# ArisKonidaris/OMLDM

Hardware: AMD Instinct MI355X
Metric: training examples/sec (whole node) + p50 predict latency, linear SVM 1/2/4/8 GPU (higher is better)
Workload: dtype fp32

## Files before the change

csrc/kernels/linear_scan3.hip:

```cpp
#include "common.h"
#include "hash_dev.h"
#include "seq_common.h"

#include <mutex>
#include <unordered_map>

namespace omldm {

typedef float f32x4 __attribute__((ext_vector_type(4)));

namespace s3 {
constexpr int CH = 64;
#ifndef OMLDM_S3_NH
#define OMLDM_S3_NH 11
#endif
constexpr int NH = OMLDM_S3_NH;
constexpr int NT = 64 * (NH + 1);
constexpr int WPE = (NH + 1 + 3) / 4;
constexpr int NHA = NH;
constexpr int GS = CH + 4;
constexpr int MAXF = 32;
constexpr int NF = (MAXF + NHA - 1) / NHA;
constexpr int KNMAX = 32;
constexpr int NJ = (KNMAX + NHA - 1) / NHA;
// ... 762 lines not shown
  const int n = cb.lidcount[s];
  const float sc = cb.inv_p * (cb.sig ? cb.sig[s] : 1.f);
  const int* l2 = cb.l2s + (size_t)s * cb.gs;
  constexpr int FB = 8;
  for (int i0 = threadIdx.x; i0 < n; i0 += FB * s3::NT) {
    int slot[FB];
    float d[FB];
#pragma unroll
    for (int u = 0; u < FB; ++u) {
      const int i = i0 + u * s3::NT;
      slot[u] = l2[i < n ? i : 0];
    }
#pragma unroll
    for (int u = 0; u < FB; ++u) {
      const int i = i0 + u * s3::NT;
      d[u] = i < min(n, cap) ? tab[i] : 0.f;
    }
    if (n > cap) {
#pragma unroll
      for (int u = 0; u < FB; ++u) {
        const int i = i0 + u * s3::NT;
        if (i >= cap && i < n)
          d[u] = __hip_atomic_load(&ag[i - cap], __ATOMIC_RELAXED, __HIP_MEMORY_SCOPE_AGENT);
      }
    }
    if constexpr (!RARE) {
#pragma unroll
      for (int u = 0; u < FB; ++u) {
        const int i = i0 + u * s3::NT;
        const int sl = i < n ? slot[u] : 0;
        d[u] -= i < n ? (cb.wbf ? s3_w16(w, sl) : w[sl]) : 0.f;
      }
    }
#pragma unroll
    for (int u = 0; u < FB; ++u) {
      const int i = i0 + u * s3::NT;
      if (i < n && d[u] != 0.f) atomicAdd(&cb.dacc[slot[u]], sc * d[u]);
    }
  }
}

__device__ __forceinline__ void s3_spoke_end(bool tail, const int* __restrict__ slotsT, int dc,
                                             int B, int R, const S3Comb& cb,
                                             const float* __restrict__ ws,
                                             const float* __restrict__ wsd, int dn, int dim,
                                             const SeqParams& p, S3Smem& sm, int s) {
  if (tail) {
    __syncthreads();
    s3_combine_spoke(slotsT, dc, B, R, cb, sm, s, 0, 1);
  }
  s3_scan_arrive(cb, ws, wsd, dn, dim, p, sm);
}

template <int RULE, int KN, bool RARE>
__device__ __forceinline__ void s3_scan_body(
    int bid, int nblk, int tail, S3Smem& sm, float* tab,
    const int* __restrict__ slotsT, const uint32_t* __restrict__ meta, int dc, int dn,
    const void* __restrict__ yv, int B, int R, const float* __restrict__ prep, int nchs,
    const float* __restrict__ w, int dim, float* __restrict__ aglob, int cap, long long gstride,
    const S3Comb& cb, float* __restrict__ ws, float* __restrict__ wsd, const SeqParams& p,
    unsigned long long* __restrict__ rgran) {
  constexpr int PF = s3_prep_floats<KN>();
  if (bid >= cb.S_act) {
    if (RARE && bid < 2 * cb.S_act) {
      s3_rare(slotsT, dc, B, R, w, cb, rgran, sm, bid - cb.S_act);
      if (cb.inscan == 2) s3_fold_pres(meta, dc, B, R, cb, bid - cb.S_act);
      if (tail == 2) {
        __syncthreads();
        s3_combine_spoke(slotsT, dc, B, R, cb, sm, bid - cb.S_act, 0, 1);
      }
      return;
    }
    s3_combine(slotsT, dc, B, R, cb, sm, (RARE ? 2 : 1) * cb.S_act, bid, nblk, cb.cns);
    return;
  }
  const int tid = threadIdx.x;
  const int wave = __builtin_amdgcn_readfirstlane(tid >> 6), lane = tid & 63;
  const int s = bid;
  int t0, t1;
  spoke_rows(s, R, B, t0, t1);
  if (t0 >= t1) {
    if (tid < s3::WS) ws[(size_t)s * s3::WS + tid] = 0.f;
    if (tid < s3::DS) wsd[(size_t)s * s3::DS + tid] = 0.f;
    s3_scan_arrive(cb, ws, wsd, dn, dim, p, sm);
    return;
  }
  const int nch = (t1 - t0 + s3::CH - 1) / s3::CH;
  const float* P0 = prep + (size_t)s * nchs * PF;
  auto chunk_prep = [&](int k) { return P0 + (size_t)k * PF; };
  float* ag = aglob + (size_t)s * gstride;

  unsigned long long* stamps = g_s3_stamps;
  const bool dbg_gather = g_s3_debug == 1;
  unsigned long long st_acc[12] = {};
  unsigned long long st_t = stamps ? clock64() : 0;
  auto stamp = [&](int k) {
    if (stamps) {
      const unsigned long long now = clock64();
      st_acc[k] += now - st_t;
      st_t = now;
    }
  };

  if (wave == 0) {
    __builtin_amdgcn_s_setprio(3);
    float loss = 0.f, nex = 0.f, mist = 0.f, sqe = 0.f;
    float f1 = 0.f;
    float ynx = chunk_prep(0)[s3_prep_y<KN>() + lane];
    float anx = chunk_prep(0)[2 * s3::MAT + lane];
    const bool shr = p.shr != 0;
    float snx = shr ? chunk_prep(0)[s3_prep_sg<KN>() + lane] : 1.f;
    float hnx = shr ? chunk_prep(0)[s3_prep_hh<KN>() + lane] : 1.f;
    for (int k = -1; k <= nch; ++k) {
      if (k >= 0 && k < nch) {
        const int b = k & 1;
        const int row = t0 + k * s3::CH + lane;
        const bool valid = row < t1 && ynx == ynx;
        const float y = valid ? ynx : 0.f;
        const float a = valid ? anx : 0.f;
        const float sg = valid ? snx : 1.f, hh = valid ? hnx : 1.f;
        if (k + 1 < nch) {
          ynx = chunk_prep(k + 1)[s3_prep_y<KN>() + lane];
          anx = chunk_prep(k + 1)[2 * s3::MAT + lane];
          if (shr) {
            snx = chunk_prep(k + 1)[s3_prep_sg<KN>() + lane];
            hnx = chunk_prep(k + 1)[s3_prep_hh<KN>() + lane];
          }
        }
        float m0 = 0.f;
#pragma unroll
        for (int q = 0; q < s3::NHA; ++q) m0 += sm.part[b][q][lane];
        S3Cand<RULE> cf;
        float u, bc = 0.f;
        const float inv = -a;
        if constexpr (RULE == kSeqHinge) {
          bc = y * inv * hh;
          cf.lo = y < 0.f ? -p.cclip * hh : 0.f;
          cf.hi = y < 0.f ? 0.f : (y > 0.f ? p.cclip * hh : 0.f);
          u = fmaf(a * (sg * hh), m0, bc) + f1;
        } else if constexpr (RULE == kSeqEps) {
          bc = (y - p.eps) * inv * hh;
          cf.d = 2.f * p.eps * inv * hh;
          cf.lo = valid ? -p.cclip * hh : 0.f;
          cf.hi = valid ? p.cclip * hh : 0.f;
          u = fmaf(a * (sg * hh), m0, bc) + f1;
        } else if constexpr (RULE == kSeqPegasos) {
          const float T = p.tbase + (float)(row - t0);
          cf.lo = valid ? 1.f / sg : 0.f;
          cf.hi = valid ? y * hh / (p.lam * T) : 0.f;
          u = fmaf(a, m0, 0.f) + f1;
        } else {
          cf.lo = y * sg;
          cf.hi = p.lr * y * hh;
          u = m0 + f1;
        }
        const float* grow = &sm.G[b][lane][0];
        const float* xrow = &sm.X1[b ^ 1][lane][0];
        float gg[s3::CH], xx[s3::CH];
#pragma unroll
        for (int t4 = 0; t4 < s3::CH; t4 += 4) {
          const float4 g4 = *reinterpret_cast<const float4*>(grow + t4);
          const float4 x4 = *reinterpret_cast<const float4*>(xrow + t4);
          gg[t4] = g4.x, gg[t4 + 1] = g4.y, gg[t4 + 2] = g4.z, gg[t4 + 3] = g4.w;
          xx[t4] = x4.x, xx[t4 + 1] = x4.y, xx[t4 + 2] = x4.z, xx[t4 + 3] = x4.w;
        }
        stamp(8);
        float n1 = 0.f;
        auto chain = [&](auto step) {
#pragma unroll
          for (int t = 0; t < s3::CH; ++t) {
            const float ct = readlane_f(step(u), t);
            u = fmaf(ct, gg[t], u);
            n1 = fmaf(ct, xx[t], n1);
            asm volatile("" : "+v"(u), "+v"(n1));
          }
        };
        if constexpr (RULE == kSeqLogistic) {
          if (!shr) {
            const float lo2 = y * 1.44269504088896341f;
            chain([&](float v) {
              return __builtin_amdgcn_rcpf(1.f + __builtin_amdgcn_exp2f(lo2 * v));
            });
          } else {
            chain([&](float v) { return cf(v, p, y); });
          }
        } else {
          chain([&](float v) { return cf(v, p, y); });
        }
        stamp(9);
        const float c = cf(u, p, y);
        sm.cb[b][lane] = c;
        if (row < t1 && cb.inscan != 1)
          __hip_atomic_store((s3_gu64*)(cb.gran + row),
                             ((unsigned long long)cb.epoch << 32) | __float_as_uint(c),
                             __ATOMIC_RELAXED, __HIP_MEMORY_SCOPE_AGENT);
        if (valid) {
          float m;
          if constexpr (RULE == kSeqLogistic) m = sg * u;
          else if constexpr (RULE == kSeqPegasos) m = sg * y * u;
          else m = inv > 0.f ? (bc - u) * __builtin_amdgcn_rcpf(inv * hh) : 0.f;
          seq_stats<RULE>(m, y, p, loss, mist, sqe);
          nex += 1.f;
        }
        f1 = n1;
      }
      stamp(0);
      __syncthreads();
      stamp(1);
    }
    if (stamps && lane == 0)
      for (int q = 0; q < 12; ++q)
        if (q < 2 || q >= 8) atomicAdd(&stamps[(size_t)s * 16 + q], st_acc[q]);
    loss = wave_sum(loss);
    nex = wave_sum(nex);
    mist = wave_sum(mist);
    sqe = wave_sum(sqe);
    if (lane == 0) {
      float* wr = ws + (size_t)s * s3::WS;
      wr[0] = loss;
      wr[1] = nex;
      wr[2] = mist;
      wr[3] = sqe;
      wr[4] = 1.f;
      wr[5] = 0.f;
      wr[6] = 0.f;
      wr[7] = 0.f;
    }
    if (cb.inscan) s3_inscan_flush<RARE>(cb, tab, ag, cap, w, s);
    s3_spoke_end(tail == 1, slotsT, dc, B, R, cb, ws, wsd, dn, dim, p, sm, s);
    return;
  }

  const int q = wave - 1, r = lane;
  const int swave = g_s3_debug >= 16 ? g_s3_debug - 16 : 1;
  if (g_s3_hprio) {
    if (q >= 7) __builtin_amdgcn_s_setprio(2);
    else if (q >= 3) __builtin_amdgcn_s_setprio(1);
  }
  const int qd = g_s3_dense_order ? s3::NHA - 1 - q : q;
  const int kd = dn + (p.bias ? 1 : 0);
  const int hl = q * 64 + lane;
  const bool inscan = cb.inscan != 0, inscan1 = cb.inscan == 1;
  const uint32_t tmask = inscan ? s3::F_TAB : s3::F_SCAT;
  const float isc = inscan1 ? cb.inv_p * (cb.sig ? cb.sig[s] : 1.f) : 0.f;
  float wn[s3::NJ], w0[s3::NJ];
#pragma unroll
  for (int i = 0; i < s3::NJ; ++i) {
    const int j = qd + s3::NHA * i;
    const int jw = j < dn ? j : dim - 1;
    const float wj = cb.wbf ? s3_w16(w, jw) : w[jw];
    w0[i] = (j < KN && (j < dn || (p.bias && j == dn))) ? wj : 0.f;
    wn[i] = w0[i];
  }
  constexpr int NV4 = (2 * s3::MAT / 4 + 64 * s3::NHA - 1) / (64 * s3::NHA);
  struct Set {
    int cs[s3::NF];
    uint32_t cm[s3::NF];
    float g[s3::NF];
    f32x4 v[NV4];
    float xs[s3::NJ], xc[s3::NJ];
    unsigned long long rg;
  };
  uint32_t p1[s3::NF], p2[s3::NF];
  const unsigned long long want = (unsigned long long)cb.epoch;
  bool dead = false;
  auto load_rare = [&](int ch) -> unsigned long long {
    const int row = t0 + ch * s3::CH + r;
    const bool ok = RARE && q == 0 && ch >= 0 && ch < nch && row < t1;
    return ok ? __hip_atomic_load((s3_gu64*)(rgran + row), __ATOMIC_RELAXED,
                                  __HIP_MEMORY_SCOPE_AGENT)
              : (want << 32);
  };
  auto load_words = [&](int ch, Set& S) {
    if constexpr (RARE) {
      S.rg = load_rare(ch);
#pragma unroll
      for (int i = 0; i < s3::NF; ++i) {
        const int f = q + s3::NHA * i;
        const int row = t0 + ch * s3::CH + r;
        const bool ok = ch >= 0 && ch < nch && f < dc && row < t1;
        const uint32_t mm = meta[ok ? (size_t)f * B + row : 0];
        S.cm[i] = ok ? mm : 0u;
        S.cs[i] = ok && (mm & (s3::F_TG | s3::F_INIT)) ? 0 : -1;
      }
      return;
    }
#pragma unroll
    for (int i = 0; i < s3::NF; ++i) {
      const int f = q + s3::NHA * i;
      const int row = t0 + ch * s3::CH + r;
      const bool ok = ch >= 0 && ch < nch && f < dc && row < t1;
      const size_t at = ok ? (size_t)f * B + row : 0;
      const int sl = slotsT[at];
      const uint32_t mm = meta[at];
      S.cs[i] = ok ? sl : -1;
      S.cm[i] = ok ? mm : 0u;
    }
  };
  auto issue_gathers = [&](Set& S) {
    if constexpr (RARE) return;
    if (cb.wbf) {
#pragma unroll
      for (int i = 0; i < s3::NF; ++i) {
        const bool glob = !RARE && S.cs[i] != -1 && !(S.cm[i] & s3::F_TG);
        S.g[i] = s3_w16(w, (glob && !dbg_gather) ? (S.cs[i] & 0x7fffffff) : 0);
      }
      return;
    }
#pragma unroll
    for (int i = 0; i < s3::NF; ++i) {
      const bool glob = !RARE && S.cs[i] != -1 && !(S.cm[i] & s3::F_TG);
      S.g[i] = w[(glob && !dbg_gather) ? (S.cs[i] & 0x7fffffff) : 0];
    }
  };
  auto issue_staging = [&](int ch, Set& S) {
#pragma unroll
    for (int u = 0; u < NV4; ++u) {
      const int i = min(hl + 64 * s3::NHA * u, 2 * s3::MAT / 4 - 1);
      const int mtx = i >> 10, e = i & 1023;
      const int kc = max(0, min(ch + mtx, nch - 1));
      S.v[u] = reinterpret_cast<const f32x4*>(chunk_prep(kc) + mtx * s3::MAT)[e];
    }
  };
  constexpr int NJK = (KN + s3::NHA - 1) / s3::NHA;
  auto load_dense = [&](int ch, float* xd) {
#pragma unroll
    for (int i = 0; i < NJK; ++i) {
      const int j = qd + s3::NHA * i;
      const bool ok = j < KN && ch >= 0 && ch < nch;
      const int jc = j < KN ? j : 0, cc = max(0, min(ch, nch - 1));
      const float v = chunk_prep(cc)[2 * s3::MAT + s3::CH + jc * s3::CH + r];
      xd[i] = ok ? v : 0.f;
    }
  };
  auto body = [&](auto spill_tag, int k, Set& CUR, Set& NXT) {
    constexpr bool SPILL = decltype(spill_tag)::value;
    const int cn = k + 1, ks = k - 1;
    if (wave == swave) stamp(7);
    load_words(cn + 1, NXT);
    issue_staging(cn + 1, NXT);
    load_dense(ks + 1, NXT.xs);
    load_dense(cn + 1, NXT.xc);
    if (wave == swave) stamp(3);
    if (ks >= 0) {
      const float cv = sm.cb[ks & 1][r];
#pragma unroll
      for (int i = 0; i < s3::NF; ++i) {
        const uint32_t m = p2[i];
        const bool sc = (m & tmask) != 0u && cv != 0.f;
        const bool dr = inscan1 && (m & s3::F_PRES) != 0u && cv != 0.f;
        if (__builtin_amdgcn_ballot_w64(sc || dr) == 0ull) continue;
        const int lid = (int)(m >> s3::LID_SHIFT);
        const float val = (m & s3::F_SIGN) ? -cv : cv;
        if (dr) atomicAdd(&cb.dacc[lid], val * isc);
        if (sc) {
          if constexpr (SPILL) {
            if (lid < cap) atomicAdd(&tab[lid], val);
            else atomicAdd(&ag[lid - cap], val);
          } else {
            atomicAdd(&tab[lid], val);
          }
        }
      }
#pragma unroll
      for (int i = 0; i < NJK; ++i) {
        const int j = qd + s3::NHA * i;
        if (j < kd) wn[i] += wave_sum(cv * CUR.xs[i]);
      }
    }
    if (wave == swave) stamp(6);
    if (cn < nch) {
      float base = 0.f;
#pragma unroll
      for (int i = 0; i < NJK; ++i) base = fmaf(CUR.xc[i], wn[i], base);
      if constexpr (RARE) {
        if (q == 0) {
          for (unsigned spins = 0;
               __builtin_amdgcn_ballot_w64((CUR.rg >> 32) != want) != 0ull;) {
            if (dead || ++spins > s3::SPIN_MAX) {
              if (!dead && r == 0) atomicExch(&g_s3_comb_err, 2);
              dead = true;
              break;
            }
            __builtin_amdgcn_s_sleep(1);
            CUR.rg = load_rare(cn);
          }
          base += (CUR.rg >> 32) == want ? __uint_as_float((uint32_t)CUR.rg) : 0.f;
        }
      }
      if constexpr (!SPILL) {
        float tv[s3::NF];
#pragma unroll
        for (int i = 0; i < s3::NF; ++i) {
          const uint32_t m = CUR.cm[i];
          const bool tg = CUR.cs[i] != -1 && (m & s3::F_TG);
          tv[i] = 0.f;
          if (tg) tv[i] = tab[(int)(m >> s3::LID_SHIFT)];
        }
#pragma unroll
        for (int i = 0; i < s3::NF; ++i) {
          const uint32_t m = CUR.cm[i];
          const bool here = CUR.cs[i] != -1;
          const bool tg = here && (m & s3::F_TG), init = here && !tg && (m & s3::F_INIT);
          const float val = tg ? tv[i] : (RARE ? 0.f : CUR.g[i]);
          if (init) tab[(int)(m >> s3::LID_SHIFT)] = val;
          if (here && (!RARE || tg)) base += (m & s3::F_SIGN) ? -val : val;
        }
      }
#pragma unroll
      for (int i = 0; SPILL && i < s3::NF; ++i) {
        const uint32_t m = CUR.cm[i];
        const bool here = CUR.cs[i] != -1;
        const int lid = (int)(m >> s3::LID_SHIFT);
        const bool tg = here && (m & s3::F_TG), init = here && !tg && (m & s3::F_INIT);
        float val = RARE ? 0.f : CUR.g[i];
        if (!SPILL || __builtin_amdgcn_ballot_w64((tg || init) && lid >= cap) == 0ull) {
          if (tg) val = tab[lid];
          if (init) tab[lid] = val;
        } else if constexpr (SPILL) {
          if (tg) val = lid < cap ? tab[lid] : __hip_atomic_load(&ag[lid - cap], __ATOMIC_RELAXED,
                                                                 __HIP_MEMORY_SCOPE_WORKGROUP);
          if (init) {
            if (lid < cap) tab[lid] = val;
            else __hip_atomic_store(&ag[lid - cap], val, __ATOMIC_RELAXED,
                                    __HIP_MEMORY_SCOPE_WORKGROUP);
          }
          asm volatile("s_waitcnt vmcnt(0)" ::: "memory");
        }
        if (here && (!RARE || tg)) base += (m & s3::F_SIGN) ? -val : val;
      }
      sm.part[cn & 1][q][r] = base;
    }
    if (wave == swave) stamp(4);
#pragma unroll
    for (int u = 0; u < NV4; ++u) {
      const int i = hl + 64 * s3::NHA * u;
      const int mtx = i >> 10, e = i & 1023;
      if (i < 2 * s3::MAT / 4 && cn + mtx < nch) {
        const int row = e >> 4, col = (e & 15) * 4;
        float* dst = mtx == 0 ? &sm.G[cn & 1][row][col] : &sm.X1[(cn + 1) & 1][row][col];
        *reinterpret_cast<f32x4*>(dst) = CUR.v[u];
      }
    }
    issue_gathers(NXT);
#pragma unroll
    for (int i = 0; i < s3::NF; ++i) {
      p2[i] = p1[i];
      p1[i] = CUR.cm[i];
    }
    if (wave == swave) stamp(5);
    __syncthreads();
  };

  Set A, Bs;
#pragma unroll
  for (int i = 0; i < s3::NF; ++i) p1[i] = p2[i] = 0u;
  load_words(0, A);
  issue_staging(0, A);
  load_dense(-2, A.xs);
  load_dense(0, A.xc);
  issue_gathers(A);
  if (cb.lidcount[s] <= cap) {
    for (int k = -1; k <= nch; k += 2) {
      body(S3Tag<false>{}, k, A, Bs);
      if (k + 1 <= nch) body(S3Tag<false>{}, k + 1, Bs, A);
    }
  } else {
    for (int k = -1; k <= nch; k += 2) {
      body(S3Tag<true>{}, k, A, Bs);
      if (k + 1 <= nch) body(S3Tag<true>{}, k + 1, Bs, A);
    }
  }
  if (stamps && lane == 0 && wave == swave)
    for (int k = 2; k < 8; ++k) atomicAdd(&stamps[(size_t)s * 16 + k], st_acc[k]);
#pragma unroll
  for (int i = 0; i < s3::NJ; ++i) {
    const int j = qd + s3::NHA * i;
    if (lane == 0 && j < KN) wsd[(size_t)s * s3::DS + j] = wn[i] - w0[i];
  }
  if (q == 0 && lane >= KN && lane < s3::DS) wsd[(size_t)s * s3::DS + lane] = 0.f;
  if (cb.inscan) s3_inscan_flush<RARE>(cb, tab, ag, cap, w, s);
  s3_spoke_end(tail == 1, slotsT, dc, B, R, cb, ws, wsd, dn, dim, p, sm, s);
}

constexpr int kS3MaxPipes = 16;
struct S3Pipe {
  const float* w;
  float* aglob;
  float* ws;
  float* wsd;
  unsigned long long* rgran;
  S3Comb cb;
  SeqParams p;
};
struct S3Pipes {
  int M;
  int ncomb;
  int tail;
  const unsigned long long* wflag;
  unsigned long long wepoch;
  S3Pipe pipe[kS3MaxPipes];
};

__global__ void s3_signal_kernel(unsigned long long* flag, unsigned long long epoch) {
  if (threadIdx.x == 0)
    __hip_atomic_store(flag, epoch, __ATOMIC_RELEASE, __HIP_MEMORY_SCOPE_AGENT);
}

__device__ __forceinline__ void s3_wait_prep(const unsigned long long* flag,
                                             unsigned long long epoch) {
  if (flag == nullptr) return;
  if (threadIdx.x == 0) {
    for (unsigned spins = 0;
         __hip_atomic_load(flag, __ATOMIC_RELAXED, __HIP_MEMORY_SCOPE_AGENT) < epoch;) {
      if (++spins > s3::SPIN_MAX) {
        atomicExch(&g_s3_comb_err, 3);
        break;
      }
      __builtin_amdgcn_s_sleep(2);
    }
    __builtin_amdgcn_fence(__ATOMIC_ACQUIRE, "agent");
  }
  __syncthreads();
}

template <int RULE, int KN, bool RARE>
__global__ __launch_bounds__(s3::NT, s3::WPE) __attribute__((amdgpu_waves_per_eu(s3::WPE, s3::WPE))) void s3_scan_kernel(
    const int* __restrict__ slotsT, const uint32_t* __restrict__ meta, int dc, int dn,
    const void* __restrict__ yv, int B, int R, const float* __restrict__ prep, int nchs,
    int dim, int cap, long long gstride, int S_act, S3Pipes pp) {
  __shared__ S3Smem sm;
  extern __shared__ float tab[];
  const int nblk = s3_nper(S_act, RARE, pp.ncomb, pp.pipe[0].cb.cns);
  const int pi = (int)blockIdx.x / nblk, local = (int)blockIdx.x % nblk;
  s3_wait_prep(pp.wflag, pp.wepoch);
  int bid;
  if (RARE && local < S_act) bid = S_act + local;
  else if (RARE && local < 2 * S_act) bid = local - S_act;
  else bid = local;
  const S3Pipe& P = pp.pipe[pi];
  s3_scan_body<RULE, KN, RARE>(bid, nblk, pp.tail, sm, tab, slotsT, meta,
                               dc, dn, yv, B, R, prep, nchs, P.w, dim, P.aglob, cap, gstride,
                               P.cb, P.ws, P.wsd, P.p, P.rgran);
}

__device__ void s3_dense_body(const float* __restrict__ ws,
                              const float* __restrict__ wsd, const float* __restrict__ sig,
                              int S_act, int dn, int dim, int bias, float inv_p,
                              float* __restrict__ dacc,
                              double* __restrict__ cum) {
  const int tid = threadIdx.x;
  const bool bad = __hip_atomic_load(&g_s3_comb_err, __ATOMIC_RELAXED, __HIP_MEMORY_SCOPE_AGENT) != 0;
  for (int i = tid; i < dn; i += 256) {
    float v = 0.f;
    for (int s = 0; s < S_act; ++s) v += wsd[(size_t)s * s3::DS + i] * (sig ? sig[s] : 1.f);
    dacc[i] = v * inv_p;
  }
  if (tid == 0) {
    float v = 0.f, a = 0.f;
    if (bias)
      for (int s = 0; s < S_act; ++s) v += wsd[(size_t)s * s3::DS + dn] * (sig ? sig[s] : 1.f);
    for (int s = 0; s < S_act; ++s) a += sig ? sig[s] : 1.f;
    dacc[dim - 1] = v * inv_p;
    dacc[dim] = a * inv_p;
    dacc[dim + 1] = bad ? -1e30f : (float)S_act * inv_p;
  }
  if (cum && !bad && tid < 6 && tid != 4) {
    double t = 0.0;
    for (int s = 0; s < S_act; ++s) t += (double)ws[(size_t)s * s3::WS + tid];
    cum[tid] += t;
  }
}

namespace s3 {
constexpr int SB = 4096;
constexpr int SH = 4096;
constexpr int SPROBE = 8;
}

__global__ __launch_bounds__(256) void s3_tail_kernel(const float* __restrict__ ws,
                                                      const float* __restrict__ wsd,
                                                      const float* __restrict__ sig, int S_act,
                                                      int dn, int dim, int bias, float inv_p,
                                                      float* __restrict__ dacc,
                                                      double* __restrict__ cum) {
  s3_dense_body(ws, wsd, sig, S_act, dn, dim, bias, inv_p, dacc, cum);
}

__global__ __launch_bounds__(256) void s3_scatter_kernel(const int* __restrict__ slotsT,
                                                         const unsigned long long* __restrict__ gran, int B,
                                                         int n_rows, float inv_p,
                                                         float* __restrict__ dacc, int dc,
                                                         const float* __restrict__ ws,
                                                         const float* __restrict__ wsd, int S_act,
                                                         int dn, int dim, int bias,
                                                         double* __restrict__ cum, int R,
// ... 543 lines not shown
      float v = 0.f;
      for (int s = 0; s < S_act; ++s) v += wsd[((size_t)s * K + c) * s3::DS + j];
      const int key = j < dn ? j : dim - 1;
      dacc[(size_t)c * dim + key] += v;
    }
    if (tid < 3) {
      float t = 0.f;
      for (int s = 0; s < S_act; ++s) t += ws[(size_t)s * s3::WS + tid];
      stats[tid] += t;
    }
    if (tid == 3) stats[3] += (float)S_act;
    return;
  }
  __shared__ int hk[s3::SH];
  __shared__ float hv[s3::SH];
  const int f = blockIdx.y, tid = threadIdx.x;
  const int r0 = blockIdx.x * s3::SB, r1 = min(n_rows, r0 + s3::SB);
  for (int i = tid; i < s3::SH; i += 256) {
    hk[i] = -1;
    hv[i] = 0.f;
  }
  __syncthreads();
  const int* col = slotsT + (size_t)f * B;
  auto add = [&](int key, float val) {
    uint32_t at = ((uint32_t)key * 0x9E3779B1u) >> (32 - 12);
    for (int probe = 0; probe < s3::SPROBE; ++probe) {
      const int prev = atomicCAS(&hk[at], -1, key);
      if (prev == -1 || prev == key) {
        atomicAdd(&hv[at], val);
        return;
      }
      at = (at + 1) & (s3::SH - 1);
    }
    atomicAdd(&dacc[key], val);
  };
  for (int row = r0 + tid; row < r1; row += 256) {
    const int v = col[row];
    const float t = tau[row];
    if (v == -1 || t == 0.f) continue;
    const int slot = v & 0x7fffffff;
    const float val = v < 0 ? -t : t;
    const float yf = load_y(yv, row, y8);
    const int yc = (yf == yf && yf >= 0.f && yf < (float)nclass) ? (int)yf : -1;
    if (yc >= 0) add(yc * dim + slot, val);
    if (rr[row] >= 0) add(rr[row] * dim + slot, -val);
  }
  __syncthreads();
  for (int i = tid; i < s3::SH; i += 256) {
    const int key = hk[i];
    if (key != -1) atomicAdd(&dacc[key], hv[i]);
  }
}

template <int RULE, int KN, bool RARE>
static int s3_launch_scan_t(const int* slotsT, const uint32_t* meta, int dc, int dn, const void* y,
                            int B, int R, int S_act, const float* prep, int nchs, int dim, int cap,
                            long long gstride, const S3Pipes& pp, hipStream_t st) {
  static bool attr_set = false;
  if (!attr_set) {
    hipFuncSetAttribute(reinterpret_cast<const void*>(&s3_scan_kernel<RULE, KN, RARE>),
                        hipFuncAttributeMaxDynamicSharedMemorySize,
                        160 * 1024 - (int)sizeof(S3Smem));
    attr_set = true;
  }
  const int nblk = pp.M * s3_nper(S_act, RARE, pp.ncomb, pp.pipe[0].cb.cns);
  hipLaunchKernelGGL((s3_scan_kernel<RULE, KN, RARE>), dim3(nblk), dim3(s3::NT),
                     (size_t)(cap + 64) * sizeof(float), st, slotsT, meta, dc, dn, y, B, R, prep,
                     nchs, dim, cap, gstride, S_act, pp);
  return (int)hipGetLastError();
}

template <int KN>
static int s3_launch_scan(int rule, bool rare, const int* slotsT, const uint32_t* meta, int dc,
                          int dn, const void* y, int B, int R, int S_act, const float* prep,
                          int nchs, int dim, int cap, long long gstride, const S3Pipes& pp,
                          hipStream_t st) {
#define OMLDM_S3L(RL, RA) \
  return s3_launch_scan_t<RL, KN, RA>(slotsT, meta, dc, dn, y, B, R, S_act, prep, nchs, dim, cap, \
                                      gstride, pp, st)
  if (rare) {
    if (rule == kSeqHinge) OMLDM_S3L(kSeqHinge, true);
    if (rule == kSeqEps) OMLDM_S3L(kSeqEps, true);
    if (rule == kSeqPegasos) OMLDM_S3L(kSeqPegasos, true);
    OMLDM_S3L(kSeqLogistic, true);
  }
  if (rule == kSeqHinge) OMLDM_S3L(kSeqHinge, false);
  if (rule == kSeqEps) OMLDM_S3L(kSeqEps, false);
  if (rule == kSeqPegasos) OMLDM_S3L(kSeqPegasos, false);
  OMLDM_S3L(kSeqLogistic, false);
#undef OMLDM_S3L
}

}

using namespace omldm;

namespace {
int s3_sact(int B, int R, int S) {
  const long long sact = ((long long)B + R - 1) / R;
  return sact < S ? (int)sact : S;
}
int s3_kn(int dn, int bias) { return dn + (bias ? 1 : 0) <= 16 ? 16 : 32; }
constexpr size_t kFlagsLds = (size_t)s3::HCAP * 12;
}

static int g_s3_cap_override = -1;

static int g_s3_mode = 4;
static int g_s3_inscan = 1;
OMLDM_API void omldm_scan3_set_inscan(int v) { g_s3_inscan = v; }
OMLDM_API void omldm_scan3_set_mode(int m) { g_s3_mode = m == 3 ? 3 : 4; }
OMLDM_API int omldm_scan3_get_mode() { return g_s3_mode; }

OMLDM_API int omldm_scan3_lds_cap() {
  const int hw = (int)((160 * 1024 - sizeof(S3Smem)) / sizeof(float)) - 64;
  return g_s3_cap_override >= 0 && g_s3_cap_override < hw ? g_s3_cap_override : hw;
}

OMLDM_API void omldm_scan3_set_cap(int cap) { g_s3_cap_override = cap; }

static int g_s3_gram_valu = 0;
OMLDM_API void omldm_scan3_set_gram_valu(int v) { g_s3_gram_valu = v; }
OMLDM_API int omldm_scan3_set_gram_ablate(int v) {
  return (int)hipMemcpyToSymbol(HIP_SYMBOL(g_s3_gram_ablate), &v, sizeof(v));
}

static int g_s3_comb = 1;
OMLDM_API void omldm_scan3_set_comb(int v) { g_s3_comb = v < 0 ? 0 : (v > 3 ? 3 : v); }
static int g_s3_form = 0;
// ... 273 lines not shown
  for (int m = 0; m < M; ++m) {
    const S3Ws Wm = s3_ws(ptrs + 8 * m);
    if (ncomb > 0 || tail || tailm || inscan) {
      if (!arrive[m])
        hipLaunchKernelGGL(s3_tail_kernel, dim3(1), dim3(256), 0, st, Wm.ws, Wm.wsd, sig, S_act,
                           dn, dim, bias, inv_p[m], dacc[m], cum[m]);
      continue;
    }
    const int n_rows = (int)((long long)S_act * R < B ? (long long)S_act * R : B);
    const int nblk = (n_rows + s3::SB - 1) / s3::SB;
    hipLaunchKernelGGL(s3_scatter_kernel, dim3(nblk > 0 ? nblk : 1, dc + (arrive[m] ? 0 : 1)),
                       dim3(256), 0, st, W0.slotsT, Wm.gran, B, n_rows, inv_p[m], dacc[m], dc,
                       Wm.ws, Wm.wsd, S_act, dn, dim, bias, cum[m], R, sig);
  }
  return (int)hipGetLastError();
}

OMLDM_API int omldm_scan3_run(const float* w, int dn, int dc, const void* y, int y8, int B, int R,
                              int S, float* dacc, int dim, double* cum, int rule, int variant,
                              float C, float eps, float lr, float inv_p, int bias,
                              long long span_in, void* const* ptrs, int part, int parts,
                              int flags, unsigned epoch, void* arrive, int shr, float lam,
                              float tbase, void* stream) {
  if (part != 0) return 0;
  (void)parts;
  return s3_run_impl(1, &w, &dacc, &cum, &C, &eps, &lr, &inv_p, ptrs, &epoch, &arrive, dn, dc, y,
                     y8, B, R, S, dim, rule, variant, bias, span_in, flags, shr, &lam, &tbase,
                     (hipStream_t)stream);
}

OMLDM_API int omldm_scan3_run_multi(int M, const float* const* w, float* const* dacc,
                                    double* const* cum, const float* C, const float* eps,
                                    const float* lr, const float* inv_p, void* const* ptrs,
                                    const unsigned* epoch, void* const* arrive, int dn, int dc,
                                    const void* y, int y8, int B, int R, int S, int dim,
                                    int rule, int variant, int bias, long long span_in, int flags,
                                    int shr, const float* lam, const float* tbase, void* stream) {
  return s3_run_impl(M, w, dacc, cum, C, eps, lr, inv_p, ptrs, epoch, arrive, dn, dc, y, y8, B, R,
                     S, dim, rule, variant, bias, span_in, flags, shr, lam, tbase,
                     (hipStream_t)stream);
}

OMLDM_API int omldm_scan3_max_pipes() { return kS3MaxPipes; }

OMLDM_API int omldm_scan3_part_bounds(int dim, int dn, int dc, long long span_in, int part,
                                      int parts, long long* lohi) {
  (void)dn, (void)dc, (void)span_in, (void)parts;
  lohi[0] = part == 0 ? 0 : (long long)dim + 2;
  lohi[1] = (long long)dim + 2;
  return 0;
}

OMLDM_API int omldm_scan3_hprio(int v) {
  return (int)hipMemcpyToSymbol(HIP_SYMBOL(g_s3_hprio), &v, sizeof(v));
}

OMLDM_API int omldm_scan3_dense_order(int v) {
  return (int)hipMemcpyToSymbol(HIP_SYMBOL(g_s3_dense_order), &v, sizeof(v));
}

OMLDM_API int omldm_scan3_debug(int v) {
  return (int)hipMemcpyToSymbol(HIP_SYMBOL(g_s3_debug), &v, sizeof(v));
}

OMLDM_API int omldm_scan3mc_debug(void* buf) {
  return (int)hipMemcpyToSymbol(HIP_SYMBOL(g_s3mc_dbg), &buf, sizeof(buf));
}

OMLDM_API int omldm_scan3_stamps(void* buf) {
  return (int)hipMemcpyToSymbol(HIP_SYMBOL(g_s3_stamps), &buf, sizeof(buf));
}

template <int K>
static int s3mc_cap() {
  return (int)((160 * 1024 - sizeof(S3McSmem<K>)) / sizeof(float)) / K * K;
}
OMLDM_API int omldm_scan3mc_lds_cap(int K) {
  switch (K) {
    case 2: return s3mc_cap<2>();
    case 4: return s3mc_cap<4>();
    case 8: return s3mc_cap<8>();
    default: return s3mc_cap<16>();
  }
}
OMLDM_API long long omldm_scan3mc_spill_floats(int R, int dc, int K) {
  return ((long long)R * dc / 2 + 64) * K;
}

template <int K, int KN>
static int s3mc_launch(const S3Ws& W, int dc, int dn, int bias, int B, int R, int S_act,
                       int nchs, int dim, long long gstride, const S3McArgs& A, hipStream_t st) {
  const int cap = omldm_scan3mc_lds_cap(K);
  static bool attr_set = false;
  if (!attr_set) {
    hipFuncSetAttribute(reinterpret_cast<const void*>(&s3mc_scan_kernel<K, KN>),
                        hipFuncAttributeMaxDynamicSharedMemorySize,
                        160 * 1024 - (int)sizeof(S3McSmem<K>));
    attr_set = true;
  }
  hipLaunchKernelGGL((s3mc_scan_kernel<K, KN>), dim3(S_act), dim3(s3::NT),
                     (size_t)cap * sizeof(float), st, W.slotsT, W.meta, W.lidcount, dc, dn, bias,
                     B, R, W.prep, nchs, dim, cap, gstride, A);
  return (int)hipGetLastError();
}

OMLDM_API int omldm_scan3mc_run(const float* Wt, int kp, int K, int nclass, int dn, int dc,
                                const void* y, int y8, int B, int R, int S, float* dacc, int dim,
                                float* stats, int variant, float C, int bias, void* const* ptrs,
                                float* ws, float* wsd, float* aglob, float* tau, int* rr,
                                void* stream) {
  if (S <= 0 || B <= 0) return 0;
  if ((K != 2 && K != 4 && K != 8 && K != 16) || nclass < 2 || nclass > K || kp < K) return -2;
  if (!omldm_scan3_fits(dn, dc, R, bias)) return -3;
  hipStream_t st = (hipStream_t)stream;
  const S3Ws W = s3_ws(ptrs);
  const int S_act = s3_sact(B, R, S);
  const int nchs = (R + s3::CH - 1) / s3::CH;
  const long long gstride = (long long)R * dc / 2 + 64;
  const S3McArgs A{Wt, kp, nclass, variant, variant == 1 ? C : INFINITY, ws, wsd, aglob, tau, rr};
  const bool k16 = s3_kn(dn, bias) == 16;
  int e;
  if (K == 2)
// ... 20 lines not shown
```

Before: 343.4 million.

## Specialize scan kernel for interior chunks and compile out debug probes

Adds a PROBE template flag so the stamp, debug, priority and order hooks are compiled out of the default kernel, with a probe instantiation chosen on the host only when those hooks are enabled. The hub loop is templated on a form (spill, edge, general, parity), so interior chunks skip the bounds checks, the ballot skip test and the dense-residual add, and use precomputed staging offsets and feature bases. Wave 0 now hoists its LDS reads of partials and G/X tiles ahead of the candidate setup, with an explicit waitcnt and scheduling barriers. This is meant to cut instruction and register overhead in the serial scan at the cost of more template instantiations and code size.

```diff
diff --git a/csrc/kernels/linear_scan3.hip b/csrc/kernels/linear_scan3.hip
--- a/csrc/kernels/linear_scan3.hip
+++ b/csrc/kernels/linear_scan3.hip
@@ -838,7 +838,13 @@
   s3_scan_arrive(cb, ws, wsd, dn, dim, p, sm);
 }
 
-template <int RULE, int KN, bool RARE>
+template <bool SPILL_, bool EDGE_, bool GEN_, int PAR_>
+struct S3Form {
+  static constexpr bool SPILL = SPILL_, EDGE = EDGE_, GEN = GEN_;
+  static constexpr int PAR = PAR_;
+};
+
+template <int RULE, int KN, bool RARE, bool PROBE>
 __device__ __forceinline__ void s3_scan_body(
     int bid, int nblk, int tail, S3Smem& sm, float* tab,
     const int* __restrict__ slotsT, const uint32_t* __restrict__ meta, int dc, int dn,
@@ -876,15 +882,17 @@
   auto chunk_prep = [&](int k) { return P0 + (size_t)k * PF; };
   float* ag = aglob + (size_t)s * gstride;
 
-  unsigned long long* stamps = g_s3_stamps;
-  const bool dbg_gather = g_s3_debug == 1;
+  unsigned long long* stamps = PROBE ? g_s3_stamps : nullptr;
+  const bool dbg_gather = PROBE && g_s3_debug == 1;
   unsigned long long st_acc[12] = {};
-  unsigned long long st_t = stamps ? clock64() : 0;
+  unsigned long long st_t = (PROBE && stamps) ? clock64() : 0;
   auto stamp = [&](int k) {
-    if (stamps) {
-      const unsigned long long now = clock64();
-      st_acc[k] += now - st_t;
-      st_t = now;
+    if constexpr (PROBE) {
+      if (stamps) {
+        const unsigned long long now = clock64();
+        st_acc[k] += now - st_t;
+        st_t = now;
+      }
     }
   };
 
@@ -897,6 +905,7 @@
     const bool shr = p.shr != 0;
     float snx = shr ? chunk_prep(0)[s3_prep_sg<KN>() + lane] : 1.f;
     float hnx = shr ? chunk_prep(0)[s3_prep_hh<KN>() + lane] : 1.f;
+    asm volatile("" : "+v"(ynx), "+v"(anx), "+v"(snx), "+v"(hnx));
     for (int k = -1; k <= nch; ++k) {
       if (k >= 0 && k < nch) {
         const int b = k & 1;
@@ -913,9 +922,25 @@
             hnx = chunk_prep(k + 1)[s3_prep_hh<KN>() + lane];
           }
         }
+        float pr[s3::NHA];
+#pragma unroll
+        for (int q = 0; q < s3::NHA; ++q) pr[q] = sm.part[b][q][lane];
+        const float* grow = &sm.G[b][lane][0];
+        const float* xrow = &sm.X1[b ^ 1][lane][0];
+        float gg[s3::CH], xx[s3::CH];
+#pragma unroll
+        for (int t4 = 0; t4 < s3::CH; t4 += 4) {
+          const float4 g4 = *reinterpret_cast<const float4*>(grow + t4);
+          const float4 x4 = *reinterpret_cast<const float4*>(xrow + t4);
+          gg[t4] = g4.x, gg[t4 + 1] = g4.y, gg[t4 + 2] = g4.z, gg[t4 + 3] = g4.w;
+          xx[t4] = x4.x, xx[t4 + 1] = x4.y, xx[t4 + 2] = x4.z, xx[t4 + 3] = x4.w;
+        }
+        __builtin_amdgcn_sched_barrier(0);
+        __builtin_amdgcn_s_waitcnt(0xC07F);
+        __builtin_amdgcn_sched_barrier(0);
         float m0 = 0.f;
 #pragma unroll
-        for (int q = 0; q < s3::NHA; ++q) m0 += sm.part[b][q][lane];
+        for (int q = 0; q < s3::NHA; ++q) m0 += pr[q];
         S3Cand<RULE> cf;
         float u, bc = 0.f;
         const float inv = -a;
@@ -940,16 +965,6 @@
           cf.hi = p.lr * y * hh;
           u = m0 + f1;
         }
-        const float* grow = &sm.G[b][lane][0];
-        const float* xrow = &sm.X1[b ^ 1][lane][0];
-        float gg[s3::CH], xx[s3::CH];
-#pragma unroll
-        for (int t4 = 0; t4 < s3::CH; t4 += 4) {
-          const float4 g4 = *reinterpret_cast<const float4*>(grow + t4);
-          const float4 x4 = *reinterpret_cast<const float4*>(xrow + t4);
-          gg[t4] = g4.x, gg[t4 + 1] = g4.y, gg[t4 + 2] = g4.z, gg[t4 + 3] = g4.w;
-          xx[t4] = x4.x, xx[t4 + 1] = x4.y, xx[t4 + 2] = x4.z, xx[t4 + 3] = x4.w;
-        }
         stamp(8);
         float n1 = 0.f;
         auto chain = [&](auto step) {
@@ -976,6 +991,7 @@
         stamp(9);
         const float c = cf(u, p, y);
         sm.cb[b][lane] = c;
+        asm volatile("" : "+v"(ynx), "+v"(anx), "+v"(snx), "+v"(hnx));
         if (row < t1 && cb.inscan != 1)
           __hip_atomic_store((s3_gu64*)(cb.gran + row),
                              ((unsigned long long)cb.epoch << 32) | __float_as_uint(c),
@@ -994,9 +1010,11 @@
       __syncthreads();
       stamp(1);
     }
-    if (stamps && lane == 0)
-      for (int q = 0; q < 12; ++q)
-        if (q < 2 || q >= 8) atomicAdd(&stamps[(size_t)s * 16 + q], st_acc[q]);
+    if constexpr (PROBE) {
+      if (stamps && lane == 0)
+        for (int q = 0; q < 12; ++q)
+          if (q < 2 || q >= 8) atomicAdd(&stamps[(size_t)s * 16 + q], st_acc[q]);
+    }
     loss = wave_sum(loss);
     nex = wave_sum(nex);
     mist = wave_sum(mist);
@@ -1018,15 +1036,20 @@
   }
 
   const int q = wave - 1, r = lane;
-  const int swave = g_s3_debug >= 16 ? g_s3_debug - 16 : 1;
-  if (g_s3_hprio) {
-    if (q >= 7) __builtin_amdgcn_s_setprio(2);
-    else if (q >= 3) __builtin_amdgcn_s_setprio(1);
-  }
-  const int qd = g_s3_dense_order ? s3::NHA - 1 - q : q;
+  int swave = 1;
+  int qd = q;
+  if constexpr (PROBE) {
+    swave = g_s3_debug >= 16 ? g_s3_debug - 16 : 1;
+    if (g_s3_hprio) {
+      if (q >= 7) __builtin_amdgcn_s_setprio(2);
+      else if (q >= 3) __builtin_amdgcn_s_setprio(1);
+    }
+    if (g_s3_dense_order) qd = s3::NHA - 1 - q;
+  }
   const int kd = dn + (p.bias ? 1 : 0);
   const int hl = q * 64 + lane;
-  const bool inscan = cb.inscan != 0, inscan1 = cb.inscan == 1;
+  const bool inscan = cb.inscan != 0, inscan1 = !RARE && cb.inscan == 1;
+  const bool wbf = cb.wbf != 0;
   const uint32_t tmask = inscan ? s3::F_TAB : s3::F_SCAT;
   const float isc = inscan1 ? cb.inv_p * (cb.sig ? cb.sig[s] : 1.f) : 0.f;
   float wn[s3::NJ], w0[s3::NJ];
@@ -1034,9 +1057,17 @@
   for (int i = 0; i < s3::NJ; ++i) {
     const int j = qd + s3::NHA * i;
     const int jw = j < dn ? j : dim - 1;
-    const float wj = cb.wbf ? s3_w16(w, jw) : w[jw];
+    const float wj = wbf ? s3_w16(w, jw) : w[jw];
     w0[i] = (j < KN && (j < dn || (p.bias && j == dn))) ? wj : 0.f;
     wn[i] = w0[i];
+  }
+  size_t fbase[s3::NF];
+  uint32_t fmask[s3::NF];
+#pragma unroll
+  for (int i = 0; i < s3::NF; ++i) {
+    const int f = q + s3::NHA * i;
+    fbase[i] = f < dc ? (size_t)f * B : 0;
+    fmask[i] = f < dc ? ~0u : 0u;
   }
   constexpr int NV4 = (2 * s3::MAT / 4 + 64 * s3::NHA - 1) / (64 * s3::NHA);
   struct Set {
@@ -1050,42 +1081,60 @@
   uint32_t p1[s3::NF], p2[s3::NF];
   const unsigned long long want = (unsigned long long)cb.epoch;
   bool dead = false;
-  auto load_rare = [&](int ch) -> unsigned long long {
-    const int row = t0 + ch * s3::CH + r;
-    const bool ok = RARE && q == 0 && ch >= 0 && ch < nch && row < t1;
-    return ok ? __hip_atomic_load((s3_gu64*)(rgran + row), __ATOMIC_RELAXED,
-                                  __HIP_MEMORY_SCOPE_AGENT)
-              : (want << 32);
+  const unsigned ur = (unsigned)r;
+  auto load_rare = [&](auto edge, int ch) -> unsigned long long {
+    if constexpr (!RARE) return want << 32;
+    if constexpr (decltype(edge)::value) {
+      const int row = t0 + ch * s3::CH + r;
+      const bool ok = q == 0 && ch >= 0 && ch < nch && row < t1;
+      return ok ? __hip_atomic_load((s3_gu64*)(rgran + row), __ATOMIC_RELAXED,
+                                    __HIP_MEMORY_SCOPE_AGENT)
+                : (want << 32);
+    } else {
+      if (q != 0) return want << 32;
+      const unsigned long long* gb = rgran + (t0 + ch * s3::CH);
+      return __hip_atomic_load((s3_gu64*)(gb + ur), __ATOMIC_RELAXED, __HIP_MEMORY_SCOPE_AGENT);
+    }
   };
-  auto load_words = [&](int ch, Set& S) {
-    if constexpr (RARE) {
-      S.rg = load_rare(ch);
-#pragma unroll
-      for (int i = 0; i < s3::NF; ++i) {
-        const int f = q + s3::NHA * i;
+  auto load_words = [&](auto edge, int ch, Set& S) {
+    constexpr bool EDGE = decltype(edge)::value;
+    if constexpr (RARE) S.rg = load_rare(edge, ch);
+#pragma unroll
+    for (int i = 0; i < s3::NF; ++i) {
+      if constexpr (EDGE) {
         const int row = t0 + ch * s3::CH + r;
-        const bool ok = ch >= 0 && ch < nch && f < dc && row < t1;
-        const uint32_t mm = meta[ok ? (size_t)f * B + row : 0];
-        S.cm[i] = ok ? mm : 0u;
-        S.cs[i] = ok && (mm & (s3::F_TG | s3::F_INIT)) ? 0 : -1;
-      }
-      return;
-    }
-#pragma unroll
-    for (int i = 0; i < s3::NF; ++i) {
-      const int f = q + s3::NHA * i;
+        const bool ok = ch >= 0 && ch < nch && row < t1;
+        const size_t at = ok ? fbase[i] + (size_t)row : 0;
+        if constexpr (!RARE) S.cs[i] = slotsT[at];
+        S.cm[i] = meta[at];
+      } else {
+        const size_t at = fbase[i] + (size_t)(t0 + ch * s3::CH);
+        if constexpr (!RARE) S.cs[i] = (slotsT + at)[ur];
+        S.cm[i] = (meta + at)[ur];
+      }
+    }
+  };
+  auto word = [&](auto edge, int ch, const Set& S, int i) -> uint32_t {
+    const uint32_t m = S.cm[i] & fmask[i];
+    if constexpr (decltype(edge)::value) {
       const int row = t0 + ch * s3::CH + r;
-      const bool ok = ch >= 0 && ch < nch && f < dc && row < t1;
-      const size_t at = ok ? (size_t)f * B + row : 0;
-      const int sl = slotsT[at];
-      const uint32_t mm = meta[at];
-      S.cs[i] = ok ? sl : -1;
-      S.cm[i] = ok ? mm : 0u;
+      return (ch >= 0 && ch < nch && row < t1) ? m : 0u;
+    } else {
+      return m;
     }
   };
-  auto issue_gathers = [&](Set& S) {
+  auto slot = [&](auto edge, int ch, const Set& S, int i) -> int {
+    const int sl = S.cs[i] | (int)~fmask[i];
+    if constexpr (decltype(edge)::value) {
+      const int row = t0 + ch * s3::CH + r;
+      return (ch >= 0 && ch < nch && row < t1) ? sl : -1;
+    } else {
+      return sl;
+    }
+  };
+  auto issue_gathers = [&](auto form, Set& S) {
     if constexpr (RARE) return;
-    if (cb.wbf) {
+    if (decltype(form)::GEN && wbf) {
 #pragma unroll
       for (int i = 0; i < s3::NF; ++i) {
         const bool glob = !RARE && S.cs[i] != -1 && !(S.cm[i] & s3::F_TG);
@@ -1099,43 +1148,68 @@
       S.g[i] = w[(glob && !dbg_gather) ? (S.cs[i] & 0x7fffffff) : 0];
     }
   };
-  auto issue_staging = [&](int ch, Set& S) {
+  unsigned voff[NV4];
+#pragma unroll
+  for (int u = 0; u < NV4; ++u) {
+    const int i = min(hl + 64 * s3::NHA * u, 2 * s3::MAT / 4 - 1);
+    const int mtx = i >> 10, e = i & 1023;
+    voff[u] = (unsigned)((mtx * (PF + s3::MAT) + e * 4) * (int)sizeof(float));
+  }
+  auto issue_staging = [&](auto edge, int ch, Set& S) {
 #pragma unroll
     for (int u = 0; u < NV4; ++u) {
-      const int i = min(hl + 64 * s3::NHA * u, 2 * s3::MAT / 4 - 1);
-      const int mtx = i >> 10, e = i & 1023;
-      const int kc = max(0, min(ch + mtx, nch - 1));
-      S.v[u] = reinterpret_cast<const f32x4*>(chunk_prep(kc) + mtx * s3::MAT)[e];
+      if constexpr (decltype(edge)::value) {
+        const int i = min(hl + 64 * s3::NHA * u, 2 * s3::MAT / 4 - 1);
+        const int mtx = i >> 10, e = i & 1023;
+        const int kc = max(0, min(ch + mtx, nch - 1));
+        S.v[u] = reinterpret_cast<const f32x4*>(chunk_prep(kc) + mtx * s3::MAT)[e];
+      } else {
+        const char* cbase = reinterpret_cast<const char*>(chunk_prep(ch));
+        S.v[u] = *reinterpret_cast<const f32x4*>(cbase + voff[u]);
+      }
     }
   };
   constexpr int NJK = (KN + s3::NHA - 1) / s3::NHA;
-  auto load_dense = [&](int ch, float* xd) {
+  auto load_dense = [&](auto edge, int ch, float* xd) {
 #pragma unroll
     for (int i = 0; i < NJK; ++i) {
       const int j = qd + s3::NHA * i;
-      const bool ok = j < KN && ch >= 0 && ch < nch;
-      const int jc = j < KN ? j : 0, cc = max(0, min(ch, nch - 1));
-      const float v = chunk_prep(cc)[2 * s3::MAT + s3::CH + jc * s3::CH + r];
-      xd[i] = ok ? v : 0.f;
+      const int jc = j < KN ? j : 0;
+      int cc = ch;
+      if constexpr (decltype(edge)::value) cc = max(0, min(ch, nch - 1));
+      const float* col = chunk_prep(cc) + (2 * s3::MAT + s3::CH + jc * s3::CH);
+      xd[i] = col[ur];
     }
   };
-  auto body = [&](auto spill_tag, int k, Set& CUR, Set& NXT) {
-    constexpr bool SPILL = decltype(spill_tag)::value;
+  auto present = [&](uint32_t m, int sl) {
+    if constexpr (RARE) return (m & (s3::F_TG | s3::F_INIT)) != 0u;
+    else return sl != -1;
+  };
+  auto body = [&](auto form, int k, Set& CUR, Set& NXT) {
+    using F = decltype(form);
+    constexpr bool SPILL = F::SPILL, EDGE = F::EDGE;
+    constexpr int PAR = F::PAR;
+    constexpr S3Tag<EDGE> edge{};
+    const bool dradd = F::GEN && inscan1;
     const int cn = k + 1, ks = k - 1;
-    if (wave == swave) stamp(7);
-    load_words(cn + 1, NXT);
-    issue_staging(cn + 1, NXT);
-    load_dense(ks + 1, NXT.xs);
-    load_dense(cn + 1, NXT.xc);
-    if (wave == swave) stamp(3);
-    if (ks >= 0) {
-      const float cv = sm.cb[ks & 1][r];
+    if constexpr (PROBE) {
+      if (wave == swave) stamp(7);
+    }
+    load_words(edge, cn + 1, NXT);
+    issue_staging(edge, cn + 1, NXT);
+    load_dense(edge, ks + 1, NXT.xs);
+    load_dense(edge, cn + 1, NXT.xc);
+    if constexpr (PROBE) {
+      if (wave == swave) stamp(3);
+    }
+    if (!EDGE || ks >= 0) {
+      const float cv = sm.cb[PAR][r];
 #pragma unroll
       for (int i = 0; i < s3::NF; ++i) {
         const uint32_t m = p2[i];
         const bool sc = (m & tmask) != 0u && cv != 0.f;
-        const bool dr = inscan1 && (m & s3::F_PRES) != 0u && cv != 0.f;
-        if (__builtin_amdgcn_ballot_w64(sc || dr) == 0ull) continue;
+        const bool dr = dradd && (m & s3::F_PRES) != 0u && cv != 0.f;
+        if (F::GEN && __builtin_amdgcn_ballot_w64(sc || dr) == 0ull) continue;
         const int lid = (int)(m >> s3::LID_SHIFT);
         const float val = (m & s3::F_SIGN) ? -cv : cv;
         if (dr) atomicAdd(&cb.dacc[lid], val * isc);
@@ -1154,11 +1228,22 @@
         if (j < kd) wn[i] += wave_sum(cv * CUR.xs[i]);
       }
     }
-    if (wave == swave) stamp(6);
-    if (cn < nch) {
+    if constexpr (PROBE) {
+      if (wave == swave) stamp(6);
+    }
+    uint32_t mw[s3::NF];
+    int sw[s3::NF];
+#pragma unroll
+    for (int i = 0; i < s3::NF; ++i) {
+      mw[i] = word(edge, cn, CUR, i);
+      if constexpr (RARE) sw[i] = 0;
+      else sw[i] = slot(edge, cn, CUR, i);
+    }
+    if (!EDGE || cn < nch) {
       float base = 0.f;
 #pragma unroll
-      for (int i = 0; i < NJK; ++i) base = fmaf(CUR.xc[i], wn[i], base);
+      for (int i = 0; i < NJK; ++i)
+        if (qd + s3::NHA * i < kd) base = fmaf(CUR.xc[i], wn[i], base);
       if constexpr (RARE) {
         if (q == 0) {
           for (unsigned spins = 0;
@@ -1169,7 +1254,7 @@
               break;
             }
             __builtin_amdgcn_s_sleep(1);
-            CUR.rg = load_rare(cn);
+            CUR.rg = load_rare(edge, cn);
           }
           base += (CUR.rg >> 32) == want ? __uint_as_float((uint32_t)CUR.rg) : 0.f;
         }
@@ -1178,15 +1263,15 @@
         float tv[s3::NF];
 #pragma unroll
         for (int i = 0; i < s3::NF; ++i) {
-          const uint32_t m = CUR.cm[i];
-          const bool tg = CUR.cs[i] != -1 && (m & s3::F_TG);
+          const uint32_t m = mw[i];
+          const bool tg = present(m, sw[i]) && (m & s3::F_TG);
           tv[i] = 0.f;
           if (tg) tv[i] = tab[(int)(m >> s3::LID_SHIFT)];
         }
 #pragma unroll
         for (int i = 0; i < s3::NF; ++i) {
-          const uint32_t m = CUR.cm[i];
-          const bool here = CUR.cs[i] != -1;
+          const uint32_t m = mw[i];
+          const bool here = present(m, sw[i]);
           const bool tg = here && (m & s3::F_TG), init = here && !tg && (m & s3::F_INIT);
           const float val = tg ? tv[i] : (RARE ? 0.f : CUR.g[i]);
           if (init) tab[(int)(m >> s3::LID_SHIFT)] = val;
@@ -1195,8 +1280,8 @@
       }
 #pragma unroll
       for (int i = 0; SPILL && i < s3::NF; ++i) {
-        const uint32_t m = CUR.cm[i];
-        const bool here = CUR.cs[i] != -1;
+        const uint32_t m = mw[i];
+        const bool here = present(m, sw[i]);
         const int lid = (int)(m >> s3::LID_SHIFT);
         const bool tg = here && (m & s3::F_TG), init = here && !tg && (m & s3::F_INIT);
         float val = RARE ? 0.f : CUR.g[i];
@@ -1215,50 +1300,69 @@
         }
         if (here && (!RARE || tg)) base += (m & s3::F_SIGN) ? -val : val;
       }
-      sm.part[cn & 1][q][r] = base;
-    }
-    if (wave == swave) stamp(4);
+      sm.part[PAR][q][r] = base;
+    }
+    if constexpr (PROBE) {
+      if (wave == swave) stamp(4);
+    }
 #pragma unroll
     for (int u = 0; u < NV4; ++u) {
       const int i = hl + 64 * s3::NHA * u;
       const int mtx = i >> 10, e = i & 1023;
-      if (i < 2 * s3::MAT / 4 && cn + mtx < nch) {
+      if (i < 2 * s3::MAT / 4 && (!EDGE || cn + mtx < nch)) {
         const int row = e >> 4, col = (e & 15) * 4;
-        float* dst = mtx == 0 ? &sm.G[cn & 1][row][col] : &sm.X1[(cn + 1) & 1][row][col];
+        float* dst = mtx == 0 ? &sm.G[PAR][row][col] : &sm.X1[PAR ^ 1][row][col];
         *reinterpret_cast<f32x4*>(dst) = CUR.v[u];
       }
     }
-    issue_gathers(NXT);
+    issue_gathers(form, NXT);
 #pragma unroll
     for (int i = 0; i < s3::NF; ++i) {
       p2[i] = p1[i];
-      p1[i] = CUR.cm[i];
-    }
-    if (wave == swave) stamp(5);
+      p1[i] = mw[i];
+    }
+    if constexpr (PROBE) {
+      if (wave == swave) stamp(5);
+    }
     __syncthreads();
   };
 
   Set A, Bs;
 #pragma unroll
   for (int i = 0; i < s3::NF; ++i) p1[i] = p2[i] = 0u;
-  load_words(0, A);
-  issue_staging(0, A);
-  load_dense(-2, A.xs);
-  load_dense(0, A.xc);
-  issue_gathers(A);
-  if (cb.lidcount[s] <= cap) {
+  load_words(S3Tag<true>{}, 0, A);
+  issue_staging(S3Tag<true>{}, 0, A);
+  load_dense(S3Tag<true>{}, -2, A.xs);
+  load_dense(S3Tag<true>{}, 0, A.xc);
+  issue_gathers(S3Form<false, true, true, 0>{}, A);
+  auto checked = [&](auto spill) {
+    constexpr bool SP = decltype(spill)::value;
     for (int k = -1; k <= nch; k += 2) {
-      body(S3Tag<false>{}, k, A, Bs);
-      if (k + 1 <= nch) body(S3Tag<false>{}, k + 1, Bs, A);
-    }
+      body(S3Form<SP, true, !RARE, 0>{}, k, A, Bs);
+      if (k + 1 <= nch) body(S3Form<SP, true, !RARE, 1>{}, k + 1, Bs, A);
+    }
+  };
+  bool general = false;
+  if constexpr (!RARE) general = inscan1 || wbf;
+  if (cb.lidcount[s] > cap) {
+    checked(S3Tag<true>{});
+  } else if (general) {
+    if constexpr (!RARE) checked(S3Tag<false>{});
   } else {
     for (int k = -1; k <= nch; k += 2) {
-      body(S3Tag<true>{}, k, A, Bs);
-      if (k + 1 <= nch) body(S3Tag<true>{}, k + 1, Bs, A);
-    }
-  }
-  if (stamps && lane == 0 && wave == swave)
-    for (int k = 2; k < 8; ++k) atomicAdd(&stamps[(size_t)s * 16 + k], st_acc[k]);
+      if (k >= 1 && k + 1 <= nch - 4) {
+        body(S3Form<false, false, false, 0>{}, k, A, Bs);
+        body(S3Form<false, false, false, 1>{}, k + 1, Bs, A);
+      } else {
+        body(S3Form<false, true, false, 0>{}, k, A, Bs);
+        if (k + 1 <= nch) body(S3Form<false, true, false, 1>{}, k + 1, Bs, A);
+      }
+    }
+  }
+  if constexpr (PROBE) {
+    if (stamps && lane == 0 && wave == swave)
+      for (int k = 2; k < 8; ++k) atomicAdd(&stamps[(size_t)s * 16 + k], st_acc[k]);
+  }
 #pragma unroll
   for (int i = 0; i < s3::NJ; ++i) {
     const int j = qd + s3::NHA * i;
@@ -1310,7 +1414,7 @@
   __syncthreads();
 }
 
-template <int RULE, int KN, bool RARE>
+template <int RULE, int KN, bool RARE, bool PROBE>
 __global__ __launch_bounds__(s3::NT, s3::WPE) __attribute__((amdgpu_waves_per_eu(s3::WPE, s3::WPE))) void s3_scan_kernel(
     const int* __restrict__ slotsT, const uint32_t* __restrict__ meta, int dc, int dn,
     const void* __restrict__ yv, int B, int R, const float* __restrict__ prep, int nchs,
@@ -1325,9 +1429,9 @@
   else if (RARE && local < 2 * S_act) bid = local - S_act;
   else bid = local;
   const S3Pipe& P = pp.pipe[pi];
-  s3_scan_body<RULE, KN, RARE>(bid, nblk, pp.tail, sm, tab, slotsT, meta,
-                               dc, dn, yv, B, R, prep, nchs, P.w, dim, P.aglob, cap, gstride,
-                               P.cb, P.ws, P.wsd, P.p, P.rgran);
+  s3_scan_body<RULE, KN, RARE, PROBE>(bid, nblk, pp.tail, sm, tab, slotsT, meta, dc, dn, yv, B, R,
+                                      prep, nchs, P.w, dim, P.aglob, cap, gstride, P.cb, P.ws,
+                                      P.wsd, P.p, P.rgran);
 }
 
 __device__ void s3_dense_body(const float* __restrict__ ws,
@@ -1977,29 +2081,42 @@
   }
 }
 
-template <int RULE, int KN, bool RARE>
+template <int RULE, int KN, bool RARE, bool PROBE = false>
 static int s3_launch_scan_t(const int* slotsT, const uint32_t* meta, int dc, int dn, const void* y,
                             int B, int R, int S_act, const float* prep, int nchs, int dim, int cap,
                             long long gstride, const S3Pipes& pp, hipStream_t st) {
   static bool attr_set = false;
   if (!attr_set) {
-    hipFuncSetAttribute(reinterpret_cast<const void*>(&s3_scan_kernel<RULE, KN, RARE>),
+    hipFuncSetAttribute(reinterpret_cast<const void*>(&s3_scan_kernel<RULE, KN, RARE, PROBE>),
                         hipFuncAttributeMaxDynamicSharedMemorySize,
                         160 * 1024 - (int)sizeof(S3Smem));
     attr_set = true;
   }
   const int nblk = pp.M * s3_nper(S_act, RARE, pp.ncomb, pp.pipe[0].cb.cns);
-  hipLaunchKernelGGL((s3_scan_kernel<RULE, KN, RARE>), dim3(nblk), dim3(s3::NT),
+  hipLaunchKernelGGL((s3_scan_kernel<RULE, KN, RARE, PROBE>), dim3(nblk), dim3(s3::NT),
                      (size_t)(cap + 64) * sizeof(float), st, slotsT, meta, dc, dn, y, B, R, prep,
                      nchs, dim, cap, gstride, S_act, pp);
   return (int)hipGetLastError();
 }
+
+static bool g_s3_probe_stamps = false;
+static int g_s3_probe_debug = 0, g_s3_probe_hprio = 0, g_s3_probe_dorder = 0;
 
 template <int KN>
 static int s3_launch_scan(int rule, bool rare, const int* slotsT, const uint32_t* meta, int dc,
                           int dn, const void* y, int B, int R, int S_act, const float* prep,
                           int nchs, int dim, int cap, long long gstride, const S3Pipes& pp,
                           hipStream_t st) {
+  if constexpr (KN == 16) {
+    if (rule == kSeqHinge && (g_s3_probe_stamps || g_s3_probe_debug || g_s3_probe_hprio ||
+                              g_s3_probe_dorder)) {
+      if (rare)
+        return s3_launch_scan_t<kSeqHinge, 16, true, true>(slotsT, meta, dc, dn, y, B, R, S_act,
+                                                           prep, nchs, dim, cap, gstride, pp, st);
+      return s3_launch_scan_t<kSeqHinge, 16, false, true>(slotsT, meta, dc, dn, y, B, R, S_act,
+                                                          prep, nchs, dim, cap, gstride, pp, st);
+    }
+  }
 #define OMLDM_S3L(RL, RA) \
   return s3_launch_scan_t<RL, KN, RA>(slotsT, meta, dc, dn, y, B, R, S_act, prep, nchs, dim, cap, \
                                       gstride, pp, st)
@@ -2379,14 +2496,17 @@
 }
 
 OMLDM_API int omldm_scan3_hprio(int v) {
+  g_s3_probe_hprio = v;
   return (int)hipMemcpyToSymbol(HIP_SYMBOL(g_s3_hprio), &v, sizeof(v));
 }
 
 OMLDM_API int omldm_scan3_dense_order(int v) {
+  g_s3_probe_dorder = v;
   return (int)hipMemcpyToSymbol(HIP_SYMBOL(g_s3_dense_order), &v, sizeof(v));
 }
 
 OMLDM_API int omldm_scan3_debug(int v) {
+  g_s3_probe_debug = v;
   return (int)hipMemcpyToSymbol(HIP_SYMBOL(g_s3_debug), &v, sizeof(v));
 }
 
@@ -2395,6 +2515,7 @@
 }
 
 OMLDM_API int omldm_scan3_stamps(void* buf) {
+  g_s3_probe_stamps = buf != nullptr;
   return (int)hipMemcpyToSymbol(HIP_SYMBOL(g_s3_stamps), &buf, sizeof(buf));
 }
 
```

Result: no change. 343.0 million, median of 3 (-0.1%).
